# nichmorgan/better-search-rag-rust

Hardware: AMD Instinct MI355X
Metric: queries/sec + p50 latency, 768-d top-10 over N vectors @1/2/4/8 GPU (higher is better)
Workload: dtype f32; 1 GPU; configs[2]: 10M x 768 f32 corpus sharded over the N GPUs, 1000 batched queries, top-10; rows_total=10000000, rows_per_gpu_rank0=10000000, queries=1000, top_k=10, dim=768, parallelism=corpus sharded over 1 GPU(s) (interval_by_rank)

## Files before the change

### better-search-rag-rust_amd/csrc/index.cpp

```cpp
#include <math.h>
#include <stdio.h>
#include <string.h>
#include <time.h>

#include <algorithm>

#include "internal.hpp"
#include "kernels.hpp"

namespace bsr {

constexpr uint32_t kMaxKForFilter = 200;

static thread_local std::string g_err;

int set_error(int code, const char* fmt, ...) {
    char buf[1024];
    va_list ap;
    va_start(ap, fmt);
    vsnprintf(buf, sizeof buf, fmt, ap);
    va_end(ap);
    g_err = buf;
    return code;
}
// ... 717 lines not shown
    bool compact;
    uint32_t tiles;
    uint32_t s_ld, n_vals;
};
static bool sample_tiles_on() {
    const char* v = getenv("BSR_SAMPLE_TILES");
    return !(v && v[0] == '0');
}
static SampleLayout sample_layout(const bsr_index* ix, uint32_t nq, uint32_t ks) {
    SampleLayout L{};
    const uint32_t BM = kFilterTile;
    L.n_s = (uint32_t)((ix->n + kSampleStride - 1) / kSampleStride);
    L.n_rt_s = (L.n_s + BM - 1) / BM;
    L.compact = L.n_s >= 32u * 8u * ks;
    const uint32_t nk = ix->op_row_bytes / 64;
    const bool qs16 = ix->op_row_bytes % 64 == 0 && nk % 2 == 0 && nk >= 2 && nk <= 12;
    if (L.compact && nq > kSkinnyMaxQ && qs16 && sample_tiles_on()) L.tiles = sample_tiles_for(ix->n);
    if (L.tiles) {
        const uint64_t last0 = ((uint64_t)(L.tiles - 1) * kSampleTileEvery + kSampleTilePhase) * 128;
        const uint64_t valid = std::min<uint64_t>(128, ix->n - last0);
        L.s_ld = 4 * L.tiles;
        L.n_vals = 4 * (L.tiles - 1) + (uint32_t)((valid + kQuantBlock - 1) / kQuantBlock);
    } else {
        L.s_ld = L.compact ? L.n_rt_s * (BM / 32) : L.n_rt_s * BM;
        L.n_vals = L.compact ? (L.n_s + 31) / 32 : L.n_s;
    }
    return L;
}

static int sample_pass(bsr_index* ix, uint32_t nq, uint32_t qpad, uint32_t k, uint64_t* smax, uint32_t ks_in = 0,
                       uint32_t cap_in = 0, const uint32_t* ks_q = nullptr) {
    BSR_TRY(filter_buffers(ix, nq, qpad, k, cap_in));
    ix->smp_tiles = 0;
    const bool skinny = nq <= kSkinnyMaxQ;
    const uint32_t cap = cap_in ? cap_in : cap_for(k);
    const uint32_t ks = ks_in ? ks_in : ks_for(k);
    const uint64_t n = ix->n;
    GemmArgs g = gemm_args(ix, qpad);
    uint32_t* status = ix->d_status;
    if (n > cap) {
        const SampleLayout L = sample_layout(ix, nq, ks);
        const uint32_t s_ld = L.s_ld, n_vals = L.n_vals;
        BSR_TRY(ix->S.ensure((size_t)qpad * s_ld * sizeof(float)));
        g.a_stride = ix->op_row_bytes;
        if (L.tiles) {
            g.a_scale_rows = kQuantBlock;
            g.n_rows = (uint32_t)n;
            g.n_rt = L.tiles;
            g.s_tiles = L.tiles;
            g.s_vals = n_vals;
            ix->smp_tiles = L.tiles;
            ix->smp_ld = s_ld;
            ix->smp_vals = n_vals;
        } else {
            g.A = ix->fop_s.as<uint8_t>();
            g.a_scale = ix->ascale_s.as<float>();
            g.a_scale_rows = kSampleScaleRows;
            g.n_rows = L.n_s;
            g.n_rt = L.n_rt_s;
        }
        g.S = ix->S.as<float>();
        g.s_ld = s_ld;
        g.s_compact = L.compact ? 1u : 0u;
        BSR_HIP(launch_timed(ix, ix->ev_sample, [&] {
            return skinny ? launch_filter_skinny_sample(g, ix->stream) : launch_filter_sample(g, ix->stream);
        }, 2));
        BSR_HIP(launch_select_tau(ix->S.as<float>(), s_ld, n_vals, nq, qpad, ix->qflags.as<uint32_t>(), ks,
                                  ix->tau.as<float>(), ix->cnt.as<uint32_t>(), status, ix->stream, smax, ks_q));
    } else {
        BSR_HIP(launch_select_tau(nullptr, 0, 0, nq, qpad, ix->qflags.as<uint32_t>(), ks, ix->tau.as<float>(),
                                  ix->cnt.as<uint32_t>(), status, ix->stream, smax, ks_q));
    }
    return BSR_OK;
}

static int emit_pass(bsr_index* ix, uint32_t nq, uint32_t qpad, uint32_t k, uint32_t cap_in = 0) {
    const bool skinny = nq <= kSkinnyMaxQ;
    GemmArgs g = emit_args(ix, nq, qpad);
    g.tau = ix->tau.as<float>();
    g.cap = cap_in ? cap_in : cap_for(k);
    g.tail = g.n_qt <= kTailCounters ? ix->cnt.as<uint32_t>() + qpad : nullptr;
    g.s_tiles = skinny ? 0u : ix->smp_tiles;
    g.S = ix->S.as<float>();
    g.s_ld = ix->smp_ld;
    g.s_vals = ix->smp_vals;
    BSR_HIP(launch_timed(ix, ix->ev_emit, [&] {
        hipError_t r = skinny ? launch_filter_skinny_emit(g, ix->stream) : launch_filter_emit(g, ix->stream);
        if (r == hipSuccess && g.s_tiles) r = launch_sample_fixup(g, ix->stream);
        return r;
    }));
    return BSR_OK;
}

static uint32_t top_layout_lab() {
    const char* lay = getenv("BSR_TOP_LAYOUT");
    return lay && lay[0] == '0' ? 0u : 2u;
}

static int top_pass(bsr_index* ix, uint32_t nq, uint32_t qpad, uint32_t k, uint32_t top) {
    BSR_TRY(filter_buffers(ix, nq, qpad, k));
    GemmArgs g = emit_args(ix, nq, qpad);
    g.cap = top;
    g.status = ix->d_status;
    g.top_layout = top_layout_lab();
    BSR_HIP(launch_timed(ix, ix->ev_emit, [&] { return launch_filter_skinny_top(g, ix->stream); }));
    return BSR_OK;
}

static RescoreArgs rescore_args(const bsr_index* ix, uint32_t nq, uint32_t k) {
    RescoreArgs r{};
    r.rows = ix->rows.as<float>();
    r.ld = ix->ld;
    r.dim = ix->dim;
    r.na = ix->na.as<float>();
    r.qf32 = ix->qf32.as<float>();
    r.nb = ix->nb.as<float>();
    r.n_items = nq;
    r.kp = kp_for(k);
    r.k = k;
    r.ebound = ix->ebound.as<float>();
    r.out_keys = ix->keys.as<uint64_t>();
// ... 729 lines not shown
            BSR_HIP(hipMemcpyAsync(h_qflags.data(), qflags.p, (size_t)nq * sizeof(uint32_t), hipMemcpyDeviceToHost, stream));
            BSR_HIP(hipStreamSynchronize(stream));
            for (uint32_t q : h_fail) {
                if (q >= nq || on_list[q]) continue;
                on_list[q] = 1;
                if (h_qflags[q] & kQueryNoApprox) ++stats.n_exact_direct;
                else ++stats.n_fallback;
            }
            stats.search_path |= BSR_PATH_MASK_LIST;
        }
    }
    BSR_TRY(run_list_scan_groups(ix, nq, k, dallow, allow_words, n_masks, on_list));
    BSR_TRY(finalize_and_read(ix, nq, k, 0, true, grp_aq.as<uint32_t>()));
    return check_queries(ix, nq);
}

bool bsr_index::gtau_eligible(uint32_t nq, uint32_t k) const {
    return loaded && nq > 0 && k >= 1 && k <= cfg.max_k && k <= kMaxKForFilter && approx_ok && n > cap_for(k) &&
           n_dead == 0;
}

int bsr_index::gtau_prepare(const float* queries, uint32_t nq, uint32_t k) {
    if (!gtau_eligible(nq, k)) return set_error(BSR_E_STATE, "global-threshold search not applicable");
    if (!queries) return set_error(BSR_E_INVALID, "null queries");
    BSR_HIP(hipSetDevice(device));
    stats = bsr_search_stats{};
    stats.n_queries = nq;
    stats.row_ebound = row_ebound;
    BSR_TRY(prepare_result(nq, k));
    const uint32_t qpad = (uint32_t)round_up(nq, kFilterTile);
    const uint32_t ks = ks_for(k);
    BSR_TRY(query_buffers(this, nq, qpad, k));
    BSR_TRY(smax.ensure((size_t)qpad * ks * sizeof(uint64_t)));
    if (!is_device_ptr(queries)) BSR_TRY(q_in.ensure((size_t)nq * dim * sizeof(float)));
    BSR_TRY(filter_buffers(this, nq, qpad, k));
    BSR_TRY(S.ensure((size_t)qpad * sample_layout(this, nq, ks).s_ld * sizeof(float)));
    gt_nq = nq;
    gt_k = k;
    gt_qpad = qpad;
    gt_ks = ks;
    return BSR_OK;
}

int bsr_index::gtau_phase_a(const float* queries, int part) {
    bsr_index* ix = this;
    const uint32_t nq = gt_nq, k = gt_k, qpad = gt_qpad;
    if (part == 1) {
        BSR_TRY(sample_pass(ix, nq, qpad, k, smax.as<uint64_t>()));
        return BSR_OK;
    }
    const float* qsrc = nullptr;
    BSR_TRY(stage_queries(ix, queries, nq, &qsrc));
    ev_begin(ix, ev_total);
    BSR_HIP(launch_query_prep(query_prep_args(ix, qsrc, nq, qpad, true), stream));
    return BSR_OK;
}

int bsr_index::gtau_phase_b(const uint64_t* g_smax, uint32_t P, uint32_t* merge_words) {
    bsr_index* ix = this;
    const uint32_t nq = gt_nq, k = gt_k, qpad = gt_qpad;
    BSR_HIP(launch_global_tau(g_smax, P, qpad, nq, gt_ks, qflags.as<uint32_t>(), tau.as<float>(), stream));
    BSR_TRY(emit_pass(ix, nq, qpad, k));
    ev_begin(ix, ev_rescore);
    RescoreArgs ra = rescore_args(ix, nq, k);
    rescore_emitted(ra, ix, cap_for(k));
    ra.excl_out = d_x;
// ... 79 lines not shown
```

### better-search-rag-rust_amd/csrc/internal.hpp

```cpp
#pragma once

#include <hip/hip_runtime.h>
#include <stdarg.h>
#include <stdint.h>

#include <atomic>

#include <string>
#include <vector>

#include "bsr.h"
#include "kernels.hpp"

namespace bsr {

int set_error(int code, const char* fmt, ...);
void clear_error();

#define BSR_HIP(call)                                                                       \
    do {                                                                                    \
        hipError_t e_ = (call);                                                             \
        if (e_ != hipSuccess)                                                               \
            return ::bsr::set_error(BSR_E_HIP, "%s failed: %s (%s:%d)", #call,              \
                                    hipGetErrorString(e_), __FILE__, __LINE__);             \
// ... 21 lines not shown
hipError_t stream_wait(hipStream_t s);
hipError_t flag_wait(const uint32_t* flag, hipStream_t s);
int select_device(int device);

static inline uint64_t round_up(uint64_t x, uint64_t m) { return (x + m - 1) / m * m; }

struct Events {
    hipEvent_t a = nullptr, b = nullptr;
    bool armed = false;
    ~Events();
    int create();
};

}

struct bsr_index {
    bsr_config cfg{};
    int device = 0;
    hipStream_t stream = nullptr;
    uint32_t dim = 0, ld = 0;
    uint64_t n = 0, n_pad = 0, global_offset = 0;
    bool loaded = false;
    bool approx_ok = false;
    uint32_t row_flags = 0;
    uint32_t op_row_bytes = 0;
    float row_ebound = 0.0f;

    bsr::DevBuf rows;
    bsr::DevBuf na;
    bsr::DevBuf fop;
    bsr::DevBuf fop_s;
    bsr::DevBuf ascale_s;
    uint32_t smp_tiles = 0, smp_ld = 0, smp_vals = 0;
    bsr::DevBuf ascale;
    bsr::DevBuf flags;

    bsr::DevBuf q_in, qf32, nb, qop, qscale, ebound, qflags, tau, S, cand, cnt, cand_rows, ncand,
        tau_excl, keys, fail, fail2, part, qids, qids_id, tmp;

    bsr::DevBuf res[2];
    uint8_t* h_res = nullptr;
    uint8_t* h_res_dev = nullptr;
    size_t h_res_bytes = 0;
    uint32_t* h_flag = nullptr;
    uint32_t* h_flag_dev = nullptr;
    bsr::DevBuf pub_ticket;
    uint32_t cur = 0;
    bool next_status_clean = false;
    size_t res_off_cnt = 0, res_off_dist = 0, res_off_idx = 0, res_off_x = 0, res_bytes = 0;
    uint32_t* d_status = nullptr;
    uint32_t* d_cnt = nullptr;
    float* d_dist = nullptr;
    uint64_t* d_idx = nullptr;
    float* d_x = nullptr;

    std::vector<uint32_t> h_qflags, h_fail;

    bsr_search_stats stats{};
    bsr_profile prof{};
    bsr::Events ev_emit, ev_sample, ev_select, ev_rescore, ev_scan, ev_total;
    int prof_level = 2;

    struct SearchKey {
        uint32_t nq = 0, k = 0;
        const float* qsrc = nullptr;
        uint64_t n = 0, gen = 0;
// ... 85 lines not shown
```

### better-search-rag-rust_amd/csrc/k_filter.hip

```cpp
#include <cstdlib>
#include "bsr_device.hpp"
#include "kernels.hpp"

#include <hip/hip_ext.h>

#include <limits.h>
#include <math.h>

#include <algorithm>
#include <type_traits>
#include <utility>

namespace bsr {

typedef __attribute__((ext_vector_type(4))) int i32x4_t;
typedef __attribute__((ext_vector_type(16))) int i32x16_t;
typedef __attribute__((address_space(3))) void lds_void_t;

constexpr int kSlots = 4;
constexpr int kSliceB = 64;
constexpr int kWCap = 256;
constexpr int kThreads = 512;

__device__ __forceinline__ void wait_vm0() { asm volatile("s_waitcnt vmcnt(0)" ::: "memory"); }
// ... 845 lines not shown
        cur_id = nxt_id;
        nxt_id = req ? __builtin_amdgcn_readfirstlane(lds_ids[t & 1]) : n2;
    }
    wait_vm0();
#ifdef BSR_FILTER_STAMPS
    if (EMIT) {
        BSR_FST(st_b);
        fst[5] = st_b - st_loop0;
        if (lane == 0)
            for (int i = 0; i < 8; ++i) atomicAdd(&g_filter_stamps[i], fst[i]);
    }
#endif
    if constexpr (EMIT) {
        if constexpr (QUEUE) {
            flush_queue();
        } else {
            flush_ring(0);
            flush_ring(1);
        }
#ifdef BSR_FILTER_COUNTERS
        if (lane == 0) {
            for (int i = 0; i < 4; ++i) atomicAdd(&g_filter_counters[i], fcnt[i]);
            if (blockIdx.x < 4096) g_filter_wg_stamps[blockIdx.x * 9 + 1 + w] = __builtin_amdgcn_s_memrealtime();
            if (blockIdx.x < 4096 && w == 0) {
                g_filter_wg_tiles[blockIdx.x * 2] = (unsigned int)fcnt[4];
                g_filter_wg_tiles[blockIdx.x * 2 + 1] = my_static;
            }
        }
#endif
    }
}


__global__ __launch_bounds__(256) void k_sample_fixup(GemmArgs p) {
    constexpr int NKM = 12, U = 4;
    const uint32_t q = blockIdx.x;
    const float tq = p.tau[q];
    if (!(tq < INFINITY)) return;
    const int tid = threadIdx.x, lane = tid & 63;
    const uint32_t w0 = __builtin_amdgcn_readfirstlane(tid >> 6) * 64;
    const uint32_t c = lane & 3, rr = lane >> 2;
    const int nk = p.row_bytes / kSliceB;
    const float sbq = p.b_scale[q];
    i32x4_t fb[NKM];
#pragma unroll
    for (int s = 0; s < NKM; ++s)
        fb[s] = s < nk ? *reinterpret_cast<const i32x4_t*>(p.B + (uint64_t)q * p.row_bytes + s * kSliceB + c * 16)
                       : i32x4_t{0, 0, 0, 0};
    auto block = [&](uint32_t j) {
        const uint32_t r0 = ((j >> 2) * kSampleTileEvery + kSampleTilePhase) * 128 + (j & 3) * 32;
        const float sc = p.a_scale[r0 / kQuantBlock];
        i32x4_t fa[2][NKM];
#pragma unroll
        for (int h = 0; h < 2; ++h) {
            const uint8_t* a = p.A + (uint64_t)(r0 + 16 * h + rr) * p.a_stride + c * 16;
#pragma unroll
            for (int s = 0; s < NKM; ++s)
                if (s < nk) fa[h][s] = *reinterpret_cast<const i32x4_t*>(a + s * kSliceB);
        }
#pragma unroll
        for (int h = 0; h < 2; ++h) {
            int acc = 0;
#pragma unroll
            for (int s = 0; s < NKM; ++s)
                if (s < nk)
#pragma unroll
                    for (int e = 0; e < 4; ++e) acc = __builtin_amdgcn_sdot4(fa[h][s][e], fb[s][e], acc, false);
            acc += (int)xor_lane32<1>((uint32_t)acc);
            acc += (int)xor_lane32<2>((uint32_t)acc);
            const float v = ((float)acc * sc) * sbq;
            const uint32_t row = r0 + 16 * h + rr;
            const bool pass = c == 0 && v >= tq && row < p.n_rows;
            const uint64_t mk = __ballot(pass);
            if (mk) {
                uint32_t gp = 0;
                if (lane == 0) gp = atomicAdd(p.cnt + q, (uint32_t)__builtin_popcountll(mk));
                gp = __builtin_amdgcn_readfirstlane(gp);
                const uint32_t pos = gp + (uint32_t)__builtin_popcountll(mk & ((1ull << lane) - 1ull));
                if (pass && pos < p.cap) p.cand[(uint64_t)q * p.cap + pos] = score_key(v, row);
            }
        }
    };
    const float* srow = p.S + (uint64_t)q * p.s_ld;
    for (uint32_t base = 0; base < p.s_vals; base += U * 256) {
        float sv[U];
#pragma unroll
        for (int u = 0; u < U; ++u) {
            const uint32_t j = base + u * 256 + tid;
            sv[u] = j < p.s_vals ? srow[j] : -INFINITY;
        }
#pragma unroll
        for (int u = 0; u < U; ++u) {
            const uint32_t j = base + u * 256 + tid;
            uint64_t m = __ballot(j < p.s_vals && sv[u] >= tq);
            while (m) {
                const uint32_t b = (uint32_t)__builtin_ctzll(m);
                m &= m - 1;
                block(base + u * 256 + w0 + b);
            }
        }
    }
}

typedef __attribute__((ext_vector_type(4))) int i32x4_acc_t;

template <bool EMIT>
__global__ __launch_bounds__(256) void k_filter_skinny(GemmArgs p) {
    constexpr int KC = 8;
    const int lane = threadIdx.x & 63, w = threadIdx.x >> 6;
    const uint32_t q = lane & 15, h = lane >> 4;
    const uint32_t nk = p.row_bytes / kSliceB;
    const uint32_t n_groups = (p.n_rows + 31) / 32;
    const uint32_t nwaves = gridDim.x * 4;
    const float sbq = p.b_scale[q];
    const float tauq = EMIT ? p.tau[q] : 0.0f;
    const uint8_t* bq = p.B + (uint64_t)q * p.row_bytes + h * 16;
    for (uint32_t g = blockIdx.x * 4 + w; g < n_groups; g += nwaves) {
        uint32_t r0 = g * 32 + q, r1 = g * 32 + 16 + q;
        r0 = r0 < p.n_rows ? r0 : p.n_rows - 1;
        r1 = r1 < p.n_rows ? r1 : p.n_rows - 1;
        const uint8_t* a0 = p.A + (uint64_t)r0 * p.a_stride + h * 16;
        const uint8_t* a1 = p.A + (uint64_t)r1 * p.a_stride + h * 16;
        i32x4_acc_t acc0 = {0, 0, 0, 0}, acc1 = {0, 0, 0, 0};
        for (uint32_t s0 = 0; s0 < nk; s0 += KC) {
            i32x4_t fa0[KC], fa1[KC], fb[KC];
#pragma unroll
            for (int s = 0; s < KC; ++s) {
                if (s0 + s < nk) {
                    fa0[s] = *reinterpret_cast<const i32x4_t*>(a0 + (s0 + s) * kSliceB);
                    fa1[s] = *reinterpret_cast<const i32x4_t*>(a1 + (s0 + s) * kSliceB);
                    fb[s] = *reinterpret_cast<const i32x4_t*>(bq + (s0 + s) * kSliceB);
                }
            }
#pragma unroll
// ... 323 lines not shown
            }
        }
    }
    if constexpr (TOP) {
#pragma unroll
        for (int off = 16; off <= 32; off <<= 1) {
            uint64_t o[4];
#pragma unroll
            for (int j = 0; j < 4; ++j) {
                const uint32_t lo = (uint32_t)__shfl_xor((int)(uint32_t)tk[j], off, kWave);
                const uint32_t hi = (uint32_t)__shfl_xor((int)(uint32_t)(tk[j] >> 32), off, kWave);
                o[j] = ((uint64_t)hi << 32) | lo;
            }
#pragma unroll
            for (int j = 0; j < 4; ++j) top4_insert(tk, o[j]);
        }
        __shared__ uint64_t wl[NW][16][4];
        if (h == 0)
#pragma unroll
            for (int j = 0; j < 4; ++j) wl[w][q][j] = tk[j];
        __syncthreads();
        if (w == 0 && h == 0) {
#pragma unroll
            for (int o = 1; o < NW; ++o)
#pragma unroll
                for (int j = 0; j < 4; ++j) top4_insert(tk, wl[o][q][j]);
            uint64_t* dst = p.cand + ((uint64_t)q * gridDim.x + blockIdx.x) * 4;
#pragma unroll
            for (int j = 0; j < 4; ++j) dst[j] = tk[j];
        }
    }
}

template <int E, bool PQ = false>
__global__ __launch_bounds__(256) void k_select_tau(const float* __restrict__ S, uint32_t s_ld,
                                                    uint32_t n_s, uint32_t nq, uint32_t qpad,
                                                    const uint32_t* __restrict__ qflags,
                                                    uint32_t ks, float* __restrict__ tau,
                                                    uint32_t* __restrict__ cnt,
                                                    uint32_t* __restrict__ status,
                                                    uint64_t* __restrict__ smax,
                                                    const uint32_t* __restrict__ ks_q) {
    __shared__ uint64_t part[4][64 * E];
    const uint32_t q = blockIdx.x;
    const int t = threadIdx.x, w = t >> 6, lane = t & 63;
    if (q == 0 && t == 0) { status[kStFail] = 0; status[kStEmitted] = 0; status[kStFail2] = 0; }
    if (q == 0)
        for (uint32_t i = t; i < 8 * kTailCounters + kGangWords; i += blockDim.x) cnt[qpad + i] = 0;
    if (q >= qpad) return;
    if (t == 0) cnt[q] = 0;
    if constexpr (PQ) ks = ks_q[q];
    if (smax && (q >= nq || (qflags[q] & kQueryNoApprox) || n_s < ks))
        for (uint32_t i = t; i < ks; i += blockDim.x) smax[(uint64_t)q * ks + i] = kKeyNone;
    if (q >= nq || (qflags[q] & kQueryNoApprox) || (PQ && ks == 0)) {
        if (t == 0) tau[q] = INFINITY;
        return;
    }
    if (n_s < ks) {
        if (t == 0) tau[q] = -INFINITY;
        return;
    }
    __shared__ float lbw[4];
    const float* s = S + (uint64_t)q * s_ld;
    const uint32_t per = (n_s + 3) / 4, lo = w * per, hi = lo + per < n_s ? lo + per : n_s;
    constexpr int B = 16;
    float m = -INFINITY;
    for (uint32_t base = lo; base < hi; base += B * kWave) {
        float v[B];
#pragma unroll
        for (int j = 0; j < B; ++j) {
            const uint32_t i = base + j * kWave + lane;
            v[j] = i < hi ? s[i] : -INFINITY;
        }
#pragma unroll
        for (int j = 0; j < B; ++j) m = fmaxf(m, v[j]);
    }
    if (ks <= (uint32_t)kWave) {
        const uint64_t sorted = wave_sort64(score_key(m, (uint32_t)lane));
        const uint64_t kth = shfl64(sorted, (int)ks - 1);
        if (lane == 0) lbw[w] = score_key_score(kth);
    } else if (lane == 0) {
        lbw[w] = -INFINITY;
    }
    __syncthreads();
    const float lb = fmaxf(fmaxf(lbw[0], lbw[1]), fmaxf(lbw[2], lbw[3]));
    WaveTopK<E> L;
    L.init();
    uint64_t thr = kKeyNone;
    for (uint32_t base = lo; base < hi; base += B * kWave) {
        float v[B];
#pragma unroll
        for (int j = 0; j < B; ++j) {
            const uint32_t i = base + j * kWave + lane;
            v[j] = i < hi ? s[i] : -INFINITY;
        }
#pragma unroll
        for (int j = 0; j < B; ++j) {
            const uint32_t i = base + j * kWave + lane;
            L.offer(v[j] >= lb ? score_key(v[j], i) : kKeyNone, (int)ks, thr);
        }
    }
#pragma unroll
    for (int e = 0; e < E; ++e) part[w][e * 64 + lane] = L.v[e];
    __syncthreads();
    if (w == 0) {
        WaveTopK<E> M;
        M.init();
        uint64_t mt = kKeyNone;
        for (int src = 0; src < 4; ++src)
#pragma unroll
            for (int e = 0; e < E; ++e) M.offer(part[src][e * 64 + lane], (int)ks, mt);
        if (lane == 0) tau[q] = score_key_score(mt);
        if (smax) M.store(smax + (uint64_t)q * ks, (int)ks);
    }
}

template <int NV, bool PQ = false>
__global__ __launch_bounds__(256) void k_select_tau_w(const float* __restrict__ S, uint32_t s_ld, uint32_t n_s,
                                                      uint32_t nq, uint32_t qpad, const uint32_t* __restrict__ qflags,
                                                      uint32_t ks, float* __restrict__ tau, uint32_t* __restrict__ cnt,
                                                      uint32_t* __restrict__ status, uint64_t* __restrict__ smax,
                                                      const uint32_t* __restrict__ ks_q) {
    const uint32_t q = blockIdx.x * 4 + (threadIdx.x >> 6);
    const int t = threadIdx.x, lane = t & 63;
    if (blockIdx.x == 0 && t == 0) { status[kStFail] = 0; status[kStEmitted] = 0; status[kStFail2] = 0; }
    if (blockIdx.x == 0)
        for (uint32_t i = t; i < 8 * kTailCounters + kGangWords; i += blockDim.x) cnt[qpad + i] = 0;
    if (q >= qpad) return;
    if (lane == 0) cnt[q] = 0;
    if constexpr (PQ) ks = ks_q[q];
    const bool none = q >= nq || (qflags[q] & kQueryNoApprox) || (PQ && ks == 0);
    if (smax && (none || n_s < ks))
        for (uint32_t i = lane; i < ks; i += kWave) smax[(uint64_t)q * ks + i] = kKeyNone;
    if (none) {
        if (lane == 0) tau[q] = INFINITY;
        return;
    }
    if (n_s < ks) {
        if (lane == 0) tau[q] = -INFINITY;
        return;
    }
    const float* s = S + (uint64_t)q * s_ld;
    float v[NV];
    float m = -INFINITY;
#pragma unroll
    for (int j = 0; j < NV; ++j) {
        const uint32_t i = j * kWave + lane;
        v[j] = i < n_s ? s[i] : -INFINITY;
    }
#pragma unroll
    for (int j = 0; j < NV; ++j) m = fmaxf(m, v[j]);
    const uint64_t sorted = wave_sort64(score_key(m, (uint32_t)lane));
    const float lb = score_key_score(shfl64(sorted, (int)ks - 1));
    WaveTopK<1> L;
    L.init();
    uint64_t thr = kKeyNone;
#pragma unroll
    for (int j = 0; j < NV; ++j) {
        const uint32_t i = j * kWave + lane;
        if (j * kWave < (int)n_s) L.offer((i < n_s && v[j] >= lb) ? score_key(v[j], i) : kKeyNone, (int)ks, thr);
    }
    if (lane == 0) tau[q] = score_key_score(thr);
    if (smax) L.store(smax + (uint64_t)q * ks, (int)ks);
}

template <int NV, bool PQ = false>
__global__ __launch_bounds__(1024) void k_select_tau_m(const float* __restrict__ S, uint32_t s_ld, uint32_t n_s,
                                                       uint32_t nq, uint32_t qpad, const uint32_t* __restrict__ qflags,
                                                       uint32_t ks, float* __restrict__ tau, uint32_t* __restrict__ cnt,
                                                       uint32_t* __restrict__ status, uint64_t* __restrict__ smax,
                                                       const uint32_t* __restrict__ ks_q) {
    constexpr int NW = 16;
    const uint32_t q = blockIdx.x;
    const int t = threadIdx.x, w = t >> 6, lane = t & 63;
    if (q == 0 && t == 0) { status[kStFail] = 0; status[kStEmitted] = 0; status[kStFail2] = 0; }
    if (q == 0)
        for (uint32_t i = t; i < 8 * kTailCounters + kGangWords; i += blockDim.x) cnt[qpad + i] = 0;
    if (q >= qpad) return;
    if (t == 0) cnt[q] = 0;
    if constexpr (PQ) ks = ks_q[q];
    const bool none = q >= nq || (qflags[q] & kQueryNoApprox) || (PQ && ks == 0);
    if (smax && (none || n_s < ks))
        for (uint32_t i = t; i < ks; i += blockDim.x) smax[(uint64_t)q * ks + i] = kKeyNone;
    if (none) {
        if (t == 0) tau[q] = INFINITY;
        return;
    }
    if (n_s < ks) {
        if (t == 0) tau[q] = -INFINITY;
        return;
    }
    __shared__ float lbw[NW];
    __shared__ uint64_t part[NW][kWave];
    const float* s = S + (uint64_t)q * s_ld;
    const uint32_t per = (n_s + NW - 1) / NW, lo = w * per, hi = lo + per < n_s ? lo + per : n_s;
    float v[NV];
    float m = -INFINITY;
#pragma unroll
    for (int j = 0; j < NV; ++j) {
        const uint32_t i = lo + j * kWave + lane;
        v[j] = i < hi ? s[i] : -INFINITY;
    }
#pragma unroll
    for (int j = 0; j < NV; ++j) m = fmaxf(m, v[j]);
    const uint64_t sorted = wave_sort64(score_key(m, (uint32_t)lane));
    const uint64_t kth = shfl64(sorted, (int)ks - 1);
    if (lane == 0) lbw[w] = score_key_score(kth);
    __syncthreads();
    float lb = lbw[0];
#pragma unroll
    for (int i = 1; i < NW; ++i) lb = fmaxf(lb, lbw[i]);
    WaveTopK<1> L;
    L.init();
    uint64_t thr = kKeyNone;
#pragma unroll
    for (int j = 0; j < NV; ++j) {
        const uint32_t i = lo + j * kWave + lane;
        if (lo + j * kWave < hi) L.offer((i < hi && v[j] >= lb) ? score_key(v[j], i) : kKeyNone, (int)ks, thr);
    }
    uint64_t* const packed = &part[0][0];
    if (lane < (int)ks) packed[w * ks + lane] = L.v[0];
    __syncthreads();
    if (w != 0) return;
    WaveTopK<1> M;
    M.init();
    uint64_t mt = kKeyNone;
    for (uint32_t b = 0; b < NW * ks; b += kWave) M.offer(b + lane < NW * ks ? packed[b + lane] : kKeyNone, (int)ks, mt);
    if (lane == 0) tau[q] = score_key_score(mt);
    if (smax) M.store(smax + (uint64_t)q * ks, (int)ks);
}

template <int E>
__global__ __launch_bounds__(256) void k_global_tau(const uint64_t* __restrict__ g, uint32_t P, uint32_t qpad,
                                                    uint32_t nq, uint32_t ks, const uint32_t* __restrict__ qflags,
                                                    float* __restrict__ tau) {
    const uint32_t q = blockIdx.x * 4 + (threadIdx.x >> 6);
    const int lane = threadIdx.x & 63;
    if (q >= qpad) return;
    if (q >= nq || (qflags[q] & kQueryNoApprox)) {
        if (lane == 0) tau[q] = INFINITY;
        return;
    }
    WaveTopK<E> L;
    L.init();
    uint64_t thr = kKeyNone;
    const uint32_t tot = P * ks;
    constexpr int NB = 8;
    for (uint32_t b = 0; b < tot; b += NB * kWave) {
        uint64_t x[NB];
#pragma unroll
        for (int u = 0; u < NB; ++u) {
            const uint32_t f = b + u * kWave + lane, r = f / ks, i = f - r * ks;
            x[u] = f < tot ? g[((uint64_t)r * qpad + q) * ks + i] : kKeyNone;
        }
#pragma unroll
        for (int u = 0; u < NB; ++u)
            if (b + u * kWave < tot) L.offer(x[u], (int)ks, thr);
    }
    if (lane == 0) tau[q] = thr == kKeyNone ? -INFINITY : score_key_score(thr);
}

template <int E>
// ... 104 lines not shown
                return;
            }
        }
        switch (nk) {
            case 2: BSR_KLAUNCH((k_filter_qs16<EMIT, 2>), g, b, s, a); return;
            case 4: BSR_KLAUNCH((k_filter_qs16<EMIT, 4>), g, b, s, a); return;
            case 6: BSR_KLAUNCH((k_filter_qs16<EMIT, 6>), g, b, s, a); return;
            case 8: BSR_KLAUNCH((k_filter_qs16<EMIT, 8>), g, b, s, a); return;
            case 10: BSR_KLAUNCH((k_filter_qs16<EMIT, 10>), g, b, s, a); return;
            default: BSR_KLAUNCH((k_filter_qs16<EMIT, 12>), g, b, s, a); return;
        }
    }
    BSR_KLAUNCH((k_filter<EMIT>), dim3(grid), dim3(kThreads), s, a);
}
hipError_t launch_filter_sample(const GemmArgs& a, hipStream_t s) {
    launch_filter<false>(a, s);
    return hipGetLastError();
}
hipError_t launch_filter_emit(const GemmArgs& a, hipStream_t s) {
    launch_filter<true>(a, s);
    return hipGetLastError();
}
hipError_t launch_filter_emit_gang(const GemmArgs& a, hipStream_t s) {
    if (a.row_bytes != 12 * kSliceB) return hipErrorInvalidValue;
    BSR_KLAUNCH((k_filter_qs16<true, 12, true>), dim3(filter_grid(a.n_qt)), dim3(512), s, a);
    return hipGetLastError();
}
hipError_t launch_sample_fixup(const GemmArgs& a, hipStream_t s) {
    const uint32_t nk = a.row_bytes / kSliceB;
    if (!a.s_tiles || !a.n_q || nk < 1 || nk > 12 || a.row_bytes % kSliceB) return hipErrorInvalidValue;
    hipLaunchKernelGGL(k_sample_fixup, dim3(a.n_q), dim3(256), 0, s, a);
    return hipGetLastError();
}
template <bool PQ>
static void launch_select_tau_pq(const float* S, uint32_t s_ld, uint32_t n_s, uint32_t nq, uint32_t qpad,
                                 const uint32_t* qflags, uint32_t ks, float* tau, uint32_t* cnt, uint32_t* status,
                                 hipStream_t s, uint64_t* smax, const uint32_t* ks_q) {
    static const int m_on = [] {
        const char* v = getenv("BSR_SELECT_TAU_M");
        return v && v[0] == '0' ? 0 : v && v[0] == '2' ? 2 : 1;
    }();
    if (m_on && ks <= kWave && (qpad <= 16 || m_on == 2) && n_s > 32 * kWave && n_s <= 16 * 16 * kWave)
        hipLaunchKernelGGL((k_select_tau_m<16, PQ>), dim3(qpad), dim3(1024), 0, s, S, s_ld, n_s, nq, qpad, qflags, ks,
                           tau, cnt, status, smax, ks_q);
    else if (ks <= kWave && n_s <= 32 * kWave && qpad % 4 == 0)
        hipLaunchKernelGGL((k_select_tau_w<32, PQ>), dim3(qpad / 4), dim3(256), 0, s, S, s_ld, n_s, nq, qpad, qflags,
                           ks, tau, cnt, status, smax, ks_q);
    else if (ks > kWave)
        hipLaunchKernelGGL((k_select_tau<2, PQ>), dim3(qpad), dim3(256), 0, s, S, s_ld, n_s, nq, qpad, qflags, ks, tau,
                           cnt, status, smax, ks_q);
    else
        hipLaunchKernelGGL((k_select_tau<1, PQ>), dim3(qpad), dim3(256), 0, s, S, s_ld, n_s, nq, qpad, qflags, ks, tau,
                           cnt, status, smax, ks_q);
}
hipError_t launch_select_tau(const float* S, uint32_t s_ld, uint32_t n_s, uint32_t nq, uint32_t qpad,
                             const uint32_t* qflags, uint32_t ks, float* tau, uint32_t* cnt, uint32_t* status,
                             hipStream_t s, uint64_t* smax, const uint32_t* ks_q) {
    if (ks > 2 * kWave || (ks_q && smax)) return hipErrorInvalidValue;
    if (ks_q) launch_select_tau_pq<true>(S, s_ld, n_s, nq, qpad, qflags, ks, tau, cnt, status, s, smax, ks_q);
    else launch_select_tau_pq<false>(S, s_ld, n_s, nq, qpad, qflags, ks, tau, cnt, status, s, smax, ks_q);
    return hipGetLastError();
}
hipError_t launch_global_tau(const uint64_t* g, uint32_t P, uint32_t qpad, uint32_t nq, uint32_t ks,
                             const uint32_t* qflags, float* tau, hipStream_t s) {
    if (ks > 2 * kWave || P == 0) return hipErrorInvalidValue;
    if (ks > kWave)
        hipLaunchKernelGGL(k_global_tau<2>, dim3(qpad / 4), dim3(256), 0, s, g, P, qpad, nq, ks, qflags, tau);
    else
        hipLaunchKernelGGL(k_global_tau<1>, dim3(qpad / 4), dim3(256), 0, s, g, P, qpad, nq, ks, qflags, tau);
    return hipGetLastError();
}
hipError_t launch_select_cand(const uint64_t* cand, const uint32_t* cnt, uint32_t cap, uint32_t nq,
                              const float* tau, uint32_t kp, uint32_t* cand_rows, uint32_t* ncand,
                              float* tau_excl, hipStream_t s) {
    const uint32_t e = (kp + 1 + 63) / 64;
#define BSR_SELECT(E)                                                                                   \
    hipLaunchKernelGGL(k_select_cand<E>, dim3(nq), dim3(64), 0, s, cand, cnt, cap, nq, tau, kp, cand_rows, \
                       ncand, tau_excl)
    switch (e) {
        case 1: BSR_SELECT(1); break;
        case 2: BSR_SELECT(2); break;
        case 3: BSR_SELECT(3); break;
        case 4: BSR_SELECT(4); break;
        case 5: BSR_SELECT(5); break;
        case 6: BSR_SELECT(6); break;
        case 7: BSR_SELECT(7); break;
        case 8: BSR_SELECT(8); break;
        case 9: BSR_SELECT(9); break;
        case 10: BSR_SELECT(10); break;
        default: return hipErrorInvalidValue;
    }
#undef BSR_SELECT
    return hipGetLastError();
// ... 4 lines not shown
```

### better-search-rag-rust_amd/csrc/kernels.hpp

```cpp
#pragma once

#include <hip/hip_runtime.h>
#include <stdint.h>

namespace bsr {

constexpr uint32_t kLdAlign = 64;
constexpr uint32_t kRowPad = 256;
constexpr uint32_t kScanQF = 8;
constexpr uint32_t kSampleStride = 32;
constexpr uint32_t kQuantBlock = 32;
constexpr uint32_t kSampleScaleRows = 128;
constexpr uint32_t kFilterTile = 256;

constexpr uint32_t kRowNonFinite = 1u;
constexpr uint32_t kRowNormOvf = 2u;
constexpr uint32_t kRowNormRange = 4u;

constexpr uint32_t kQueryNonFinite = 1u;
constexpr uint32_t kQueryNoApprox = 2u;

enum StatusWord : uint32_t { kStFail = 0, kStEmitted = 1, kStQueryFlags = 2, kStFail2 = 3, kStWords = 4 };

hipError_t launch_synth_uniform(float* out, uint64_t row0, uint64_t n_rows, uint32_t dim,
// ... 87 lines not shown
    uint64_t a_stride;
    uint32_t n_rows;
    uint32_t a_scale_rows;
    const uint8_t* B;
    uint32_t row_bytes;
    uint32_t n_rt, n_qt;
    const float* a_scale;
    const float* b_scale;
    float* S;
    uint32_t s_ld;
    uint32_t s_compact;
    const float* tau;
    uint64_t* cand;
    uint32_t* cnt;
    uint32_t cap;
    uint32_t* tail;
    uint32_t* status;
    uint32_t n_q;
    uint32_t top_layout;
    uint32_t s_tiles, s_vals;
};
constexpr uint32_t kSampleTileEvery = 32;
constexpr uint32_t kSampleTilePhase = 31;
static inline uint32_t sample_tiles_for(uint64_t n) { return (uint32_t)(((n + 127) / 128) / kSampleTileEvery); }
constexpr uint32_t kTailDiv = 8;
constexpr uint32_t kTailCounters = 64;
constexpr uint32_t kGangWords = 2 * 256;
constexpr uint32_t kGangMinTiles = 600;
constexpr int kEmitQueueDepth = 48;
hipError_t launch_filter_sample(const GemmArgs& a, hipStream_t s);
hipError_t launch_filter_emit(const GemmArgs& a, hipStream_t s);
hipError_t launch_filter_emit_gang(const GemmArgs& a, hipStream_t s);
hipError_t launch_sample_fixup(const GemmArgs& a, hipStream_t s);
constexpr uint32_t kSkinnyMaxQ = 16;
hipError_t launch_filter_skinny_sample(const GemmArgs& a, hipStream_t s);
hipError_t launch_filter_skinny_emit(const GemmArgs& a, hipStream_t s);
hipError_t launch_filter_skinny_top(const GemmArgs& a, hipStream_t s);
uint32_t skinny_top_lists(uint32_t n_rows);
bool skinny_glds_on();
constexpr uint64_t kSkinnyTopMinRows = 2u << 20;

hipError_t launch_select_tau(const float* S, uint32_t s_ld, uint32_t n_s, uint32_t nq,
                             uint32_t qpad, const uint32_t* qflags, uint32_t ks, float* tau,
                             uint32_t* cnt, uint32_t* status, hipStream_t s, uint64_t* smax = nullptr,
                             const uint32_t* ks_q = nullptr);
hipError_t launch_global_tau(const uint64_t* g, uint32_t P, uint32_t qpad, uint32_t nq, uint32_t ks,
                             const uint32_t* qflags, float* tau, hipStream_t s);
hipError_t launch_select_cand(const uint64_t* cand, const uint32_t* cnt, uint32_t cap,
                              uint32_t nq, const float* tau, uint32_t kp, uint32_t* cand_rows,
                              uint32_t* ncand, float* tau_excl, hipStream_t s);

struct RescoreArgs {
    const float* rows;
    uint32_t ld, dim;
    const float* na;
    const float* qf32;
    const float* nb;
    uint32_t n_items;
    const uint32_t* n_items_dev;
    const uint32_t* qlist;
    const uint32_t* cand_rows;
    const uint32_t* ncand;
    uint32_t kp;
    const float* tau_excl;
    const uint64_t* cand_keys;
    const uint32_t* cnt;
    uint32_t cap;
    const float* tau0;
    uint32_t sel;
    uint32_t top_w;
    const uint32_t* qflags;
    float* top_tau;
    uint32_t* top_cnt;
    uint32_t k;
    const float* ebound;
    uint64_t* out_keys;
    uint32_t* fail_cnt;
    uint32_t* fail_list;
// ... 92 lines not shown
```

Baseline: 178,400 queries/s.

## Drive sample fixup from the tau-selection key list instead of rescanning all sample values

The tau-selection kernels now record, per query, whether exactly ks sampled values are at or above the threshold, so the stored top-ks key list fully identifies the sample blocks that need fixup. A new fixup kernel then rescores only those listed blocks, one wave per key, and falls back to the full per-query scan of the sample row when the list is not known to be complete. This is meant to cut the fixup pass's linear scan over the sample scores. In exchange, select_tau does extra ballot counting and sometimes a second pass over S, and a small per-query completion buffer is added.

```diff
diff --git a/better-search-rag-rust_amd/csrc/index.cpp b/better-search-rag-rust_amd/csrc/index.cpp
--- a/better-search-rag-rust_amd/csrc/index.cpp
+++ b/better-search-rag-rust_amd/csrc/index.cpp
@@ -773,6 +773,7 @@
                        uint32_t cap_in = 0, const uint32_t* ks_q = nullptr) {
     BSR_TRY(filter_buffers(ix, nq, qpad, k, cap_in));
     ix->smp_tiles = 0;
+    ix->smp_keys = nullptr;
     const bool skinny = nq <= kSkinnyMaxQ;
     const uint32_t cap = cap_in ? cap_in : cap_for(k);
     const uint32_t ks = ks_in ? ks_in : ks_for(k);
@@ -793,6 +794,15 @@
             ix->smp_tiles = L.tiles;
             ix->smp_ld = s_ld;
             ix->smp_vals = n_vals;
+            if (!ks_in && !ks_q) {
+                if (!smax) {
+                    BSR_TRY(ix->smax.ensure((size_t)qpad * ks * sizeof(uint64_t)));
+                    smax = ix->smax.as<uint64_t>();
+                }
+                BSR_TRY(ix->smp_done.ensure((size_t)qpad * sizeof(uint32_t)));
+                ix->smp_keys = smax;
+                ix->smp_ks = ks;
+            }
         } else {
             g.A = ix->fop_s.as<uint8_t>();
             g.a_scale = ix->ascale_s.as<float>();
@@ -807,7 +817,8 @@
             return skinny ? launch_filter_skinny_sample(g, ix->stream) : launch_filter_sample(g, ix->stream);
         }, 2));
         BSR_HIP(launch_select_tau(ix->S.as<float>(), s_ld, n_vals, nq, qpad, ix->qflags.as<uint32_t>(), ks,
-                                  ix->tau.as<float>(), ix->cnt.as<uint32_t>(), status, ix->stream, smax, ks_q));
+                                  ix->tau.as<float>(), ix->cnt.as<uint32_t>(), status, ix->stream, smax, ks_q,
+                                  ix->smp_keys ? ix->smp_done.as<uint32_t>() : nullptr));
     } else {
         BSR_HIP(launch_select_tau(nullptr, 0, 0, nq, qpad, ix->qflags.as<uint32_t>(), ks, ix->tau.as<float>(),
                                   ix->cnt.as<uint32_t>(), status, ix->stream, smax, ks_q));
@@ -827,7 +838,10 @@
     g.s_vals = ix->smp_vals;
     BSR_HIP(launch_timed(ix, ix->ev_emit, [&] {
         hipError_t r = skinny ? launch_filter_skinny_emit(g, ix->stream) : launch_filter_emit(g, ix->stream);
-        if (r == hipSuccess && g.s_tiles) r = launch_sample_fixup(g, ix->stream);
+        if (r == hipSuccess && g.s_tiles)
+            r = ix->smp_keys ? launch_sample_fixup_list(g, ix->smp_keys, ix->smp_done.as<uint32_t>(), ix->smp_ks,
+                                                        ix->stream)
+                             : launch_sample_fixup(g, ix->stream);
         return r;
     }));
     return BSR_OK;
@@ -1623,6 +1637,7 @@
     const uint32_t ks = ks_for(k);
     BSR_TRY(query_buffers(this, nq, qpad, k));
     BSR_TRY(smax.ensure((size_t)qpad * ks * sizeof(uint64_t)));
+    BSR_TRY(smp_done.ensure((size_t)qpad * sizeof(uint32_t)));
     if (!is_device_ptr(queries)) BSR_TRY(q_in.ensure((size_t)nq * dim * sizeof(float)));
     BSR_TRY(filter_buffers(this, nq, qpad, k));
     BSR_TRY(S.ensure((size_t)qpad * sample_layout(this, nq, ks).s_ld * sizeof(float)));
diff --git a/better-search-rag-rust_amd/csrc/internal.hpp b/better-search-rag-rust_amd/csrc/internal.hpp
--- a/better-search-rag-rust_amd/csrc/internal.hpp
+++ b/better-search-rag-rust_amd/csrc/internal.hpp
@@ -77,6 +77,9 @@
     bsr::DevBuf fop_s;
     bsr::DevBuf ascale_s;
     uint32_t smp_tiles = 0, smp_ld = 0, smp_vals = 0;
+    const uint64_t* smp_keys = nullptr;
+    uint32_t smp_ks = 0;
+    bsr::DevBuf smp_done;
     bsr::DevBuf ascale;
     bsr::DevBuf flags;
 
diff --git a/better-search-rag-rust_amd/csrc/k_filter.hip b/better-search-rag-rust_amd/csrc/k_filter.hip
--- a/better-search-rag-rust_amd/csrc/k_filter.hip
+++ b/better-search-rag-rust_amd/csrc/k_filter.hip
@@ -901,55 +901,59 @@
 }
 
 
-__global__ __launch_bounds__(256) void k_sample_fixup(GemmArgs p) {
-    constexpr int NKM = 12, U = 4;
-    const uint32_t q = blockIdx.x;
-    const float tq = p.tau[q];
-    if (!(tq < INFINITY)) return;
+constexpr int kFixupNK = 12;
+__device__ __forceinline__ void fixup_query(const GemmArgs& p, uint32_t q, int nk, uint32_t c, i32x4_t (&fb)[kFixupNK]) {
+#pragma unroll
+    for (int s = 0; s < kFixupNK; ++s)
+        fb[s] = s < nk ? *reinterpret_cast<const i32x4_t*>(p.B + (uint64_t)q * p.row_bytes + s * kSliceB + c * 16)
+                       : i32x4_t{0, 0, 0, 0};
+}
+__device__ __forceinline__ void fixup_block(const GemmArgs& p, uint32_t q, uint32_t j, float tq, float sbq, int nk,
+                                            const i32x4_t (&fb)[kFixupNK]) {
+    constexpr int NKM = kFixupNK;
+    const int lane = threadIdx.x & 63;
+    const uint32_t c = lane & 3, rr = lane >> 2;
+    const uint32_t r0 = ((j >> 2) * kSampleTileEvery + kSampleTilePhase) * 128 + (j & 3) * 32;
+    const float sc = p.a_scale[r0 / kQuantBlock];
+    i32x4_t fa[2][NKM];
+#pragma unroll
+    for (int h = 0; h < 2; ++h) {
+        const uint8_t* a = p.A + (uint64_t)(r0 + 16 * h + rr) * p.a_stride + c * 16;
+#pragma unroll
+        for (int s = 0; s < NKM; ++s)
+            if (s < nk) fa[h][s] = *reinterpret_cast<const i32x4_t*>(a + s * kSliceB);
+    }
+#pragma unroll
+    for (int h = 0; h < 2; ++h) {
+        int acc = 0;
+#pragma unroll
+        for (int s = 0; s < NKM; ++s)
+            if (s < nk)
+#pragma unroll
+                for (int e = 0; e < 4; ++e) acc = __builtin_amdgcn_sdot4(fa[h][s][e], fb[s][e], acc, false);
+        acc += (int)xor_lane32<1>((uint32_t)acc);
+        acc += (int)xor_lane32<2>((uint32_t)acc);
+        const float v = ((float)acc * sc) * sbq;
+        const uint32_t row = r0 + 16 * h + rr;
+        const bool pass = c == 0 && v >= tq && row < p.n_rows;
+        const uint64_t mk = __ballot(pass);
+        if (mk) {
+            uint32_t gp = 0;
+            if (lane == 0) gp = atomicAdd(p.cnt + q, (uint32_t)__builtin_popcountll(mk));
+            gp = __builtin_amdgcn_readfirstlane(gp);
+            const uint32_t pos = gp + (uint32_t)__builtin_popcountll(mk & ((1ull << lane) - 1ull));
+            if (pass && pos < p.cap) p.cand[(uint64_t)q * p.cap + pos] = score_key(v, row);
+        }
+    }
+}
+__device__ __forceinline__ void fixup_scan(const GemmArgs& p, uint32_t q, float tq) {
+    constexpr int U = 4;
     const int tid = threadIdx.x, lane = tid & 63;
     const uint32_t w0 = __builtin_amdgcn_readfirstlane(tid >> 6) * 64;
-    const uint32_t c = lane & 3, rr = lane >> 2;
     const int nk = p.row_bytes / kSliceB;
     const float sbq = p.b_scale[q];
-    i32x4_t fb[NKM];
-#pragma unroll
-    for (int s = 0; s < NKM; ++s)
-        fb[s] = s < nk ? *reinterpret_cast<const i32x4_t*>(p.B + (uint64_t)q * p.row_bytes + s * kSliceB + c * 16)
-                       : i32x4_t{0, 0, 0, 0};
-    auto block = [&](uint32_t j) {
-        const uint32_t r0 = ((j >> 2) * kSampleTileEvery + kSampleTilePhase) * 128 + (j & 3) * 32;
-        const float sc = p.a_scale[r0 / kQuantBlock];
-        i32x4_t fa[2][NKM];
-#pragma unroll
-        for (int h = 0; h < 2; ++h) {
-            const uint8_t* a = p.A + (uint64_t)(r0 + 16 * h + rr) * p.a_stride + c * 16;
-#pragma unroll
-            for (int s = 0; s < NKM; ++s)
-                if (s < nk) fa[h][s] = *reinterpret_cast<const i32x4_t*>(a + s * kSliceB);
-        }
-#pragma unroll
-        for (int h = 0; h < 2; ++h) {
-            int acc = 0;
-#pragma unroll
-            for (int s = 0; s < NKM; ++s)
-                if (s < nk)
-#pragma unroll
-                    for (int e = 0; e < 4; ++e) acc = __builtin_amdgcn_sdot4(fa[h][s][e], fb[s][e], acc, false);
-            acc += (int)xor_lane32<1>((uint32_t)acc);
-            acc += (int)xor_lane32<2>((uint32_t)acc);
-            const float v = ((float)acc * sc) * sbq;
-            const uint32_t row = r0 + 16 * h + rr;
-            const bool pass = c == 0 && v >= tq && row < p.n_rows;
-            const uint64_t mk = __ballot(pass);
-            if (mk) {
-                uint32_t gp = 0;
-                if (lane == 0) gp = atomicAdd(p.cnt + q, (uint32_t)__builtin_popcountll(mk));
-                gp = __builtin_amdgcn_readfirstlane(gp);
-                const uint32_t pos = gp + (uint32_t)__builtin_popcountll(mk & ((1ull << lane) - 1ull));
-                if (pass && pos < p.cap) p.cand[(uint64_t)q * p.cap + pos] = score_key(v, row);
-            }
-        }
-    };
+    i32x4_t fb[kFixupNK];
+    fixup_query(p, q, nk, lane & 3, fb);
     const float* srow = p.S + (uint64_t)q * p.s_ld;
     for (uint32_t base = 0; base < p.s_vals; base += U * 256) {
         float sv[U];
@@ -965,10 +969,41 @@
             while (m) {
                 const uint32_t b = (uint32_t)__builtin_ctzll(m);
                 m &= m - 1;
-                block(base + u * 256 + w0 + b);
-            }
-        }
-    }
+                fixup_block(p, q, base + u * 256 + w0 + b, tq, sbq, nk, fb);
+            }
+        }
+    }
+}
+__global__ __launch_bounds__(256) void k_sample_fixup(GemmArgs p) {
+    const uint32_t q = blockIdx.x;
+    const float tq = p.tau[q];
+    if (!(tq < INFINITY)) return;
+    fixup_scan(p, q, tq);
+}
+
+__global__ __launch_bounds__(256) void k_sample_fixup_list(GemmArgs p, const uint64_t* __restrict__ keys,
+                                                           const uint32_t* __restrict__ complete, uint32_t ks) {
+    if (blockIdx.x < p.n_q) {
+        const uint32_t q = blockIdx.x;
+        const float tq = p.tau[q];
+        if (!(tq < INFINITY) || complete[q]) return;
+        fixup_scan(p, q, tq);
+        return;
+    }
+    const uint32_t slot = (blockIdx.x - p.n_q) * 4 + __builtin_amdgcn_readfirstlane(threadIdx.x >> 6);
+    if (slot >= p.n_q * ks) return;
+    const uint32_t q = slot / ks;
+    const float tq = p.tau[q];
+    const uint32_t done = complete[q];
+    const uint64_t key = keys[(uint64_t)q * ks + (slot - q * ks)];
+    if (!(tq < INFINITY) || !done) return;
+    if (key == kKeyNone || !(score_key_score(key) >= tq)) return;
+    const uint32_t j = key_row(key);
+    if (j >= p.s_vals) return;
+    const int nk = p.row_bytes / kSliceB;
+    i32x4_t fb[kFixupNK];
+    fixup_query(p, q, nk, threadIdx.x & 3, fb);
+    fixup_block(p, q, j, tq, p.b_scale[q], nk, fb);
 }
 
 typedef __attribute__((ext_vector_type(4))) int i32x4_acc_t;
@@ -1358,6 +1393,20 @@
     }
 }
 
+__device__ __forceinline__ uint32_t select_complete(const uint64_t* lists, int n_lists, int stride, int n_keys,
+                                                    uint32_t ks, float tau0) {
+    const int lane = lane_id();
+    const uint64_t last = lane < n_lists ? lists[lane * stride + (int)ks - 1] : kKeyNone;
+    const bool unsure = last != kKeyNone && !(score_key_score(last) < tau0);
+    if (__ballot(unsure)) return 2u;
+    uint32_t ge = 0;
+    for (int b = 0; b < n_keys; b += kWave) {
+        const uint64_t key = b + lane < n_keys ? lists[b + lane] : kKeyNone;
+        ge += (uint32_t)__popcll(__ballot(key != kKeyNone && score_key_score(key) >= tau0));
+    }
+    return ge == ks ? 1u : 0u;
+}
+
 template <int E, bool PQ = false>
 __global__ __launch_bounds__(256) void k_select_tau(const float* __restrict__ S, uint32_t s_ld,
                                                     uint32_t n_s, uint32_t nq, uint32_t qpad,
@@ -1366,7 +1415,8 @@
                                                     uint32_t* __restrict__ cnt,
                                                     uint32_t* __restrict__ status,
                                                     uint64_t* __restrict__ smax,
-                                                    const uint32_t* __restrict__ ks_q) {
+                                                    const uint32_t* __restrict__ ks_q,
+                                                    uint32_t* __restrict__ complete) {
     __shared__ uint64_t part[4][64 * E];
     const uint32_t q = blockIdx.x;
     const int t = threadIdx.x, w = t >> 6, lane = t & 63;
@@ -1378,6 +1428,7 @@
     if constexpr (PQ) ks = ks_q[q];
     if (smax && (q >= nq || (qflags[q] & kQueryNoApprox) || n_s < ks))
         for (uint32_t i = t; i < ks; i += blockDim.x) smax[(uint64_t)q * ks + i] = kKeyNone;
+    if (complete && t == 0) complete[q] = 0;
     if (q >= nq || (qflags[q] & kQueryNoApprox) || (PQ && ks == 0)) {
         if (t == 0) tau[q] = INFINITY;
         return;
@@ -1387,6 +1438,7 @@
         return;
     }
     __shared__ float lbw[4];
+    __shared__ uint32_t fin[3];
     const float* s = S + (uint64_t)q * s_ld;
     const uint32_t per = (n_s + 3) / 4, lo = w * per, hi = lo + per < n_s ? lo + per : n_s;
     constexpr int B = 16;
@@ -1438,7 +1490,30 @@
             for (int e = 0; e < E; ++e) M.offer(part[src][e * 64 + lane], (int)ks, mt);
         if (lane == 0) tau[q] = score_key_score(mt);
         if (smax) M.store(smax + (uint64_t)q * ks, (int)ks);
-    }
+        if (complete) {
+            const uint32_t d = select_complete(&part[0][0], 4, 64 * E, 4 * 64 * E, ks, score_key_score(mt));
+            if (lane == 0) {
+                fin[0] = d;
+                fin[1] = __float_as_uint(score_key_score(mt));
+                fin[2] = 0;
+            }
+        }
+    }
+    if (!complete) return;
+    __syncthreads();
+    if (fin[0] != 2u) {
+        if (t == 0) complete[q] = fin[0];
+        return;
+    }
+    const float tau0 = __uint_as_float(fin[1]);
+    uint32_t ge = 0;
+    for (uint32_t base = lo; base < hi; base += kWave) {
+        const uint32_t i = base + lane;
+        ge += (uint32_t)__popcll(__ballot(i < hi && s[i] >= tau0));
+    }
+    if (lane == 0) atomicAdd(&fin[2], ge);
+    __syncthreads();
+    if (t == 0) complete[q] = fin[2] == ks ? 1u : 0u;
 }
 
 template <int NV, bool PQ = false>
@@ -1446,7 +1521,8 @@
                                                       uint32_t nq, uint32_t qpad, const uint32_t* __restrict__ qflags,
                                                       uint32_t ks, float* __restrict__ tau, uint32_t* __restrict__ cnt,
                                                       uint32_t* __restrict__ status, uint64_t* __restrict__ smax,
-                                                      const uint32_t* __restrict__ ks_q) {
+                                                      const uint32_t* __restrict__ ks_q,
+                                                      uint32_t* __restrict__ complete) {
     const uint32_t q = blockIdx.x * 4 + (threadIdx.x >> 6);
     const int t = threadIdx.x, lane = t & 63;
     if (blockIdx.x == 0 && t == 0) { status[kStFail] = 0; status[kStEmitted] = 0; status[kStFail2] = 0; }
@@ -1458,6 +1534,7 @@
     const bool none = q >= nq || (qflags[q] & kQueryNoApprox) || (PQ && ks == 0);
     if (smax && (none || n_s < ks))
         for (uint32_t i = lane; i < ks; i += kWave) smax[(uint64_t)q * ks + i] = kKeyNone;
+    if (complete && lane == 0 && (none || n_s < ks)) complete[q] = 0;
     if (none) {
         if (lane == 0) tau[q] = INFINITY;
         return;
@@ -1488,6 +1565,16 @@
     }
     if (lane == 0) tau[q] = score_key_score(thr);
     if (smax) L.store(smax + (uint64_t)q * ks, (int)ks);
+    if (complete) {
+        const float tau0 = score_key_score(thr);
+        uint32_t ge = 0;
+#pragma unroll
+        for (int j = 0; j < NV; ++j) {
+            const uint32_t i = j * kWave + lane;
+            ge += (uint32_t)__popcll(__ballot(i < n_s && v[j] >= tau0));
+        }
+        if (lane == 0) complete[q] = ge == ks ? 1u : 0u;
+    }
 }
 
 template <int NV, bool PQ = false>
@@ -1495,7 +1582,8 @@
                                                        uint32_t nq, uint32_t qpad, const uint32_t* __restrict__ qflags,
                                                        uint32_t ks, float* __restrict__ tau, uint32_t* __restrict__ cnt,
                                                        uint32_t* __restrict__ status, uint64_t* __restrict__ smax,
-                                                       const uint32_t* __restrict__ ks_q) {
+                                                       const uint32_t* __restrict__ ks_q,
+                                                       uint32_t* __restrict__ complete) {
     constexpr int NW = 16;
     const uint32_t q = blockIdx.x;
     const int t = threadIdx.x, w = t >> 6, lane = t & 63;
@@ -1508,6 +1596,7 @@
     const bool none = q >= nq || (qflags[q] & kQueryNoApprox) || (PQ && ks == 0);
     if (smax && (none || n_s < ks))
         for (uint32_t i = t; i < ks; i += blockDim.x) smax[(uint64_t)q * ks + i] = kKeyNone;
+    if (complete && t == 0) complete[q] = 0;
     if (none) {
         if (t == 0) tau[q] = INFINITY;
         return;
@@ -1517,6 +1606,7 @@
         return;
     }
     __shared__ float lbw[NW];
+    __shared__ uint32_t fin[3];
     __shared__ uint64_t part[NW][kWave];
     const float* s = S + (uint64_t)q * s_ld;
     const uint32_t per = (n_s + NW - 1) / NW, lo = w * per, hi = lo + per < n_s ? lo + per : n_s;
@@ -1547,13 +1637,40 @@
     uint64_t* const packed = &part[0][0];
     if (lane < (int)ks) packed[w * ks + lane] = L.v[0];
     __syncthreads();
-    if (w != 0) return;
-    WaveTopK<1> M;
-    M.init();
-    uint64_t mt = kKeyNone;
-    for (uint32_t b = 0; b < NW * ks; b += kWave) M.offer(b + lane < NW * ks ? packed[b + lane] : kKeyNone, (int)ks, mt);
-    if (lane == 0) tau[q] = score_key_score(mt);
-    if (smax) M.store(smax + (uint64_t)q * ks, (int)ks);
+    if (w != 0 && !complete) return;
+    if (w == 0) {
+        WaveTopK<1> M;
+        M.init();
+        uint64_t mt = kKeyNone;
+        for (uint32_t b = 0; b < NW * ks; b += kWave)
+            M.offer(b + lane < NW * ks ? packed[b + lane] : kKeyNone, (int)ks, mt);
+        if (lane == 0) tau[q] = score_key_score(mt);
+        if (smax) M.store(smax + (uint64_t)q * ks, (int)ks);
+        if (complete) {
+            const uint32_t d = select_complete(packed, NW, (int)ks, (int)(NW * ks), ks, score_key_score(mt));
+            if (lane == 0) {
+                fin[0] = d;
+                fin[1] = __float_as_uint(score_key_score(mt));
+                fin[2] = 0;
+            }
+        }
+    }
+    if (!complete) return;
+    __syncthreads();
+    if (fin[0] != 2u) {
+        if (t == 0) complete[q] = fin[0];
+        return;
+    }
+    const float tau0 = __uint_as_float(fin[1]);
+    uint32_t ge = 0;
+#pragma unroll
+    for (int j = 0; j < NV; ++j) {
+        const uint32_t i = lo + j * kWave + lane;
+        ge += (uint32_t)__popcll(__ballot(i < hi && v[j] >= tau0));
+    }
+    if (lane == 0) atomicAdd(&fin[2], ge);
+    __syncthreads();
+    if (t == 0) complete[q] = fin[2] == ks ? 1u : 0u;
 }
 
 template <int E>
@@ -1724,33 +1841,42 @@
     hipLaunchKernelGGL(k_sample_fixup, dim3(a.n_q), dim3(256), 0, s, a);
     return hipGetLastError();
 }
+hipError_t launch_sample_fixup_list(const GemmArgs& a, const uint64_t* keys, const uint32_t* complete, uint32_t ks,
+                                    hipStream_t s) {
+    const uint32_t nk = a.row_bytes / kSliceB;
+    if (!a.s_tiles || !a.n_q || nk < 1 || nk > 12 || a.row_bytes % kSliceB || !keys || !complete || !ks || ks > 2 * kWave)
+        return hipErrorInvalidValue;
+    const uint32_t wgs = a.n_q + (a.n_q * ks + 3) / 4;
+    hipLaunchKernelGGL(k_sample_fixup_list, dim3(wgs), dim3(256), 0, s, a, keys, complete, ks);
+    return hipGetLastError();
+}
 template <bool PQ>
 static void launch_select_tau_pq(const float* S, uint32_t s_ld, uint32_t n_s, uint32_t nq, uint32_t qpad,
                                  const uint32_t* qflags, uint32_t ks, float* tau, uint32_t* cnt, uint32_t* status,
-                                 hipStream_t s, uint64_t* smax, const uint32_t* ks_q) {
+                                 hipStream_t s, uint64_t* smax, const uint32_t* ks_q, uint32_t* complete) {
     static const int m_on = [] {
         const char* v = getenv("BSR_SELECT_TAU_M");
         return v && v[0] == '0' ? 0 : v && v[0] == '2' ? 2 : 1;
     }();
     if (m_on && ks <= kWave && (qpad <= 16 || m_on == 2) && n_s > 32 * kWave && n_s <= 16 * 16 * kWave)
         hipLaunchKernelGGL((k_select_tau_m<16, PQ>), dim3(qpad), dim3(1024), 0, s, S, s_ld, n_s, nq, qpad, qflags, ks,
-                           tau, cnt, status, smax, ks_q);
+                           tau, cnt, status, smax, ks_q, complete);
     else if (ks <= kWave && n_s <= 32 * kWave && qpad % 4 == 0)
         hipLaunchKernelGGL((k_select_tau_w<32, PQ>), dim3(qpad / 4), dim3(256), 0, s, S, s_ld, n_s, nq, qpad, qflags,
-                           ks, tau, cnt, status, smax, ks_q);
+                           ks, tau, cnt, status, smax, ks_q, complete);
     else if (ks > kWave)
         hipLaunchKernelGGL((k_select_tau<2, PQ>), dim3(qpad), dim3(256), 0, s, S, s_ld, n_s, nq, qpad, qflags, ks, tau,
-                           cnt, status, smax, ks_q);
+                           cnt, status, smax, ks_q, complete);
     else
         hipLaunchKernelGGL((k_select_tau<1, PQ>), dim3(qpad), dim3(256), 0, s, S, s_ld, n_s, nq, qpad, qflags, ks, tau,
-                           cnt, status, smax, ks_q);
+                           cnt, status, smax, ks_q, complete);
 }
 hipError_t launch_select_tau(const float* S, uint32_t s_ld, uint32_t n_s, uint32_t nq, uint32_t qpad,
                              const uint32_t* qflags, uint32_t ks, float* tau, uint32_t* cnt, uint32_t* status,
-                             hipStream_t s, uint64_t* smax, const uint32_t* ks_q) {
-    if (ks > 2 * kWave || (ks_q && smax)) return hipErrorInvalidValue;
-    if (ks_q) launch_select_tau_pq<true>(S, s_ld, n_s, nq, qpad, qflags, ks, tau, cnt, status, s, smax, ks_q);
-    else launch_select_tau_pq<false>(S, s_ld, n_s, nq, qpad, qflags, ks, tau, cnt, status, s, smax, ks_q);
+                             hipStream_t s, uint64_t* smax, const uint32_t* ks_q, uint32_t* blocks_complete) {
+    if (ks > 2 * kWave || (ks_q && smax) || (blocks_complete && !smax)) return hipErrorInvalidValue;
+    if (ks_q) launch_select_tau_pq<true>(S, s_ld, n_s, nq, qpad, qflags, ks, tau, cnt, status, s, smax, ks_q, nullptr);
+    else launch_select_tau_pq<false>(S, s_ld, n_s, nq, qpad, qflags, ks, tau, cnt, status, s, smax, ks_q, blocks_complete);
     return hipGetLastError();
 }
 hipError_t launch_global_tau(const uint64_t* g, uint32_t P, uint32_t qpad, uint32_t nq, uint32_t ks,
diff --git a/better-search-rag-rust_amd/csrc/kernels.hpp b/better-search-rag-rust_amd/csrc/kernels.hpp
--- a/better-search-rag-rust_amd/csrc/kernels.hpp
+++ b/better-search-rag-rust_amd/csrc/kernels.hpp
@@ -143,6 +143,8 @@
 hipError_t launch_filter_emit(const GemmArgs& a, hipStream_t s);
 hipError_t launch_filter_emit_gang(const GemmArgs& a, hipStream_t s);
 hipError_t launch_sample_fixup(const GemmArgs& a, hipStream_t s);
+hipError_t launch_sample_fixup_list(const GemmArgs& a, const uint64_t* keys, const uint32_t* complete, uint32_t ks,
+                                    hipStream_t s);
 constexpr uint32_t kSkinnyMaxQ = 16;
 hipError_t launch_filter_skinny_sample(const GemmArgs& a, hipStream_t s);
 hipError_t launch_filter_skinny_emit(const GemmArgs& a, hipStream_t s);
@@ -154,7 +156,7 @@
 hipError_t launch_select_tau(const float* S, uint32_t s_ld, uint32_t n_s, uint32_t nq,
                              uint32_t qpad, const uint32_t* qflags, uint32_t ks, float* tau,
                              uint32_t* cnt, uint32_t* status, hipStream_t s, uint64_t* smax = nullptr,
-                             const uint32_t* ks_q = nullptr);
+                             const uint32_t* ks_q = nullptr, uint32_t* blocks_complete = nullptr);
 hipError_t launch_global_tau(const uint64_t* g, uint32_t P, uint32_t qpad, uint32_t nq, uint32_t ks,
                              const uint32_t* qflags, float* tau, hipStream_t s);
 hipError_t launch_select_cand(const uint64_t* cand, const uint32_t* cnt, uint32_t cap,
```

Measured after the change: 178,900 queries/s (median of 6 runs). About the same (+0.3%).
